# shenwei356/wfa

Hardware: AMD Instinct MI355X
Metric: aligned pairs/sec (and Gcells/s) on 1e6 synthetic 1 kbp pairs @5% error (higher is better)
Workload: dtype u32; 1 GPU; 1000000 x 1000 bp pairs/GPU @5% error, global gap-affine 4/6/2, wf-adaptive 10/50/1, seed 3; config=c3, pairs_per_gpu=1000000, length=1000, parallelism=pair-sharded x1, ranks_seen_by_collective=1, backend=none (1 GPU), collective_forced=False, status_ok=1000000, setup_steps=0, gather=none (1 GPU), gather_bytes_per_rank_step=0, packed_pairs=1000000, retried_pairs=832

## Files before the change

wfa_amd/csrc/wfa_ctx.hpp:

```cpp
#pragma once
#include "../../include/wfa_hip.h"
#include "wfa_common.hpp"

#include <algorithm>
#include <atomic>
#include <chrono>
#include <cmath>
#include <cstdio>
#include <cstdlib>
#include <cstring>
#include <deque>
#include <functional>
#include <malloc.h>
#include <mutex>
#include <new>
#include <numeric>
#include <string>
#include <thread>
#include <vector>
#include <fcntl.h>
#include <optional>
#include <sys/file.h>
#include <unistd.h>

// ... 105 lines not shown
    int64_t       opt_team_slack           = 1024;
    bool          dbg_teamc                = false;
    DevBuf        xbuf;
    int64_t       opt_team_paged           = 1;
    DevBuf        page_ctl;
    int64_t       opt_team_xcd             = 2;
    int64_t       opt_arena_poison         = 0;
    int64_t       opt_pilot                = 1;
    int64_t       opt_tail_overlap         = 1;
    int64_t       opt_overlap              = 0;
    int64_t       opt_fail_pass            = 0;
    int64_t       opt_prepack              = 0;
    int64_t       opt_narrow_long          = 0;
    DevBuf        score_out;
    DevBuf        wide_ckpt;
    DevBuf        mx_seq, mx_words;
    DevBuf        sd_ctl, sd_blk, sd_list, sd_redo;
    uint64_t      sd_n_words = 0, sd_n_listed = 0;
    DevBuf        mx_out;
    uint2        *mx_pin       = nullptr;
    size_t        mx_pin_bytes = 0;
    hipEvent_t    mx_ev[4]     = {};
    int64_t       opt_matrix_tile_cells    = 0;
    int64_t       opt_score_long_min       = 64;
    int64_t       opt_score_long_window    = 256;
    int64_t       opt_wide                 = 1;
    int64_t       opt_wide_max_len         = 2047;
    int           opt_wide_waves           = 0;
    bool          opt_wide_exact           = false;
    int64_t       opt_wide_min_pairs       = 64;
    int64_t       opt_duo                  = 1;
    int64_t       opt_duo_min_pairs        = 200000;
    bool          opt_duo_pk               = true;
    int64_t       opt_duo_short            = 0;
    int64_t       opt_duo_short_min_pairs  = 50000;
    bool          ctrl_clean               = false;
    hipStream_t   ctrl_clean_stream        = nullptr;
    hipEvent_t    ctrl_clean_ev            = nullptr;
    bool          redo_was_empty           = false;
    int64_t       opt_compact_call_bases   = 50000000;
    int64_t       opt_lane                 = 1;
    int64_t       opt_lane_pack            = 1;
    int64_t       opt_lane_min_pairs       = 32768;
    int64_t       opt_long                 = 1;
    int64_t       opt_long_min_len         = 4000;
    int64_t       opt_long_window_words    = 240;
    int64_t       opt_long_first           = 0;
    int64_t       opt_long_wave_bt         = 1;
    int64_t       opt_census               = 0;
    int64_t       opt_learn                = 1;
    uint64_t      learn_key                = 0;
    int           learn_level              = 0;
    uint32_t      learn_calls              = 0;
    uint64_t      rows_key                 = 0;
    uint32_t      rows_scale               = 1;
    uint64_t      band_key                 = 0;
    int           band_kind                = 0;
    uint32_t      band_calls               = 0;
    int64_t       opt_blk_mid              = 1;
    int64_t       opt_mem_limit            = 0;
    int           force_mode               = -1;
    const uint32_t *dbg_arena = nullptr;
    const uint4    *dbg_meta  = nullptr;
    uint64_t        dbg_words = 0, dbg_first = 0, dbg_n = 0;
    uint32_t        dbg_fmt = 0, dbg_g = 1;
    wfahip_timing timing{};
// ... 49 lines not shown
```

wfa_amd/csrc/wfa_duo.hip:

```cpp
#define WFA_NO_AUX_KERNELS 1
#include "wfa_duo.hpp"
#include "wfa_fwd.hpp"

namespace wfa {

namespace {
template <int DX, int DOE>
hipError_t go_duo(const KParams &P, uint32_t grid, size_t lds_bytes, hipStream_t st, bool census, bool pk) {
    if (pk && census)
        hipLaunchKernelGGL((wfa_duo_kernel<true, DX, DOE>), dim3(grid), dim3(64), lds_bytes, st, P);
    else if (pk)
        hipLaunchKernelGGL((wfa_duo_kernel<false, DX, DOE>), dim3(grid), dim3(64), lds_bytes, st, P);
    else if (census)
        hipLaunchKernelGGL((wfa_duo32_kernel<true, DX, DOE>), dim3(grid), dim3(64), lds_bytes, st, P);
    else
        hipLaunchKernelGGL((wfa_duo32_kernel<false, DX, DOE>), dim3(grid), dim3(64), lds_bytes, st, P);
    return hipGetLastError();
}
}

hipError_t wfa_launch_duo(int shape, const KParams &P, uint32_t grid, size_t lds_bytes, hipStream_t st, bool census, bool pk) {
    switch (shape) {
    case 0: return go_duo<2, 4>(P, grid, lds_bytes, st, census, pk);
    case 1: return go_duo<1, 3>(P, grid, lds_bytes, st, census, pk);
    case 2: return go_duo<1, 2>(P, grid, lds_bytes, st, census, pk);
    case 3: return go_duo<2, 3>(P, grid, lds_bytes, st, census, pk);
    case 4: return go_duo<2, 2>(P, grid, lds_bytes, st, census, pk);
    case 5: return go_duo<3, 3>(P, grid, lds_bytes, st, census, pk);
    }
    return hipErrorInvalidValue;
}

}
```

wfa_amd/csrc/wfa_duo.hpp:

```cpp
#pragma once
#include "wfa_blk.hpp"
#include "wfa_duo_cfg.hpp"
#include "wfa_pk16.hpp"

namespace wfa {

struct DuoRed {
#define WFA_DUO_3(opa, opb, opc)                                                                                    \
    unsigned long long sv;                                                                                          \
    asm volatile("s_nop 1\n\t" opa " %0, %0, %0 " WFA_DPP_CTL_XOR1 "\n\t" opb " %1, %1, %1 " WFA_DPP_CTL_XOR1 "\n\t" opc \
        " %2, %2, %2 " WFA_DPP_CTL_XOR1 "\n\t" opa " %0, %0, %0 " WFA_DPP_CTL_XOR2 "\n\t" opb " %1, %1, %1 "        \
        WFA_DPP_CTL_XOR2 "\n\t" opc " %2, %2, %2 " WFA_DPP_CTL_XOR2 "\n\t" opa " %0, %0, %0 " WFA_DPP_CTL_HMIR "\n\t" \
        opb " %1, %1, %1 " WFA_DPP_CTL_HMIR "\n\t" opc " %2, %2, %2 " WFA_DPP_CTL_HMIR "\n\t"                         \
        "s_and_saveexec_b64 %3, %4\n\t" opa " %0, %0, %0 " WFA_DPP_CTL_MIR "\n\t" opb " %1, %1, %1 " WFA_DPP_CTL_MIR    \
        "\n\t" opc " %2, %2, %2 " WFA_DPP_CTL_MIR "\n\ts_mov_b64 exec, %3"                                            \
        : "+v"(a), "+v"(b), "+v"(c), "=&s"(sv)                                                                      \
        : "s"(wm)                                                                                                   \
        : "scc");
#define WFA_DUO_2(opa, opb)                                                                                         \
    unsigned long long sv;                                                                                          \
    asm volatile("s_nop 1\n\t" opa " %0, %0, %0 " WFA_DPP_CTL_XOR1 "\n\t" opb " %1, %1, %1 " WFA_DPP_CTL_XOR1 "\n\ts_nop 0\n\t" \
        opa " %0, %0, %0 " WFA_DPP_CTL_XOR2 "\n\t" opb " %1, %1, %1 " WFA_DPP_CTL_XOR2 "\n\ts_nop 0\n\t" opa        \
        " %0, %0, %0 " WFA_DPP_CTL_HMIR "\n\t" opb " %1, %1, %1 " WFA_DPP_CTL_HMIR "\n\t"                            \
        "s_and_saveexec_b64 %2, %3\n\t" opa " %0, %0, %0 " WFA_DPP_CTL_MIR "\n\t" opb " %1, %1, %1 " WFA_DPP_CTL_MIR    \
        "\n\ts_mov_b64 exec, %2"                                                                                    \
        : "+v"(a), "+v"(b), "=&s"(sv)                                                                               \
        : "s"(wm)                                                                                                   \
        : "scc");
#define WFA_DUO_1(opa)                                                                                              \
    unsigned long long sv;                                                                                          \
    asm volatile("s_nop 1\n\t" opa " %0, %0, %0 " WFA_DPP_CTL_XOR1 "\n\ts_nop 1\n\t" opa " %0, %0, %0 " WFA_DPP_CTL_XOR2 \
        "\n\ts_nop 1\n\t" opa " %0, %0, %0 " WFA_DPP_CTL_HMIR "\n\t"                                                \
        "s_and_saveexec_b64 %1, %2\n\ts_nop 0\n\t" opa " %0, %0, %0 " WFA_DPP_CTL_MIR "\n\ts_mov_b64 exec, %1"       \
        : "+v"(a), "=&s"(sv)                                                                                        \
        : "s"(wm)                                                                                                   \
        : "scc");
    static WFA_DEV void min_max_min(int &a, int &b, int &c, unsigned long long wm) { WFA_DUO_3("v_min_i32_dpp", "v_max_i32_dpp", "v_min_i32_dpp") }
    static WFA_DEV void min_max(int &a, int &b, unsigned long long wm) { WFA_DUO_2("v_min_i32_dpp", "v_max_i32_dpp") }
    static WFA_DEV void max_add(int &a, int &b, unsigned long long wm) { WFA_DUO_2("v_max_i32_dpp", "v_add_u32_dpp") }
    static WFA_DEV int  max1(int a, unsigned long long wm) {
        WFA_DUO_1("v_max_i32_dpp")
        return a;
    }
    static WFA_DEV int or1(int a, unsigned long long wm) {
        WFA_DUO_1("v_or_b32_dpp")
        return a;
    }
#undef WFA_DUO_3
#undef WFA_DUO_2
#undef WFA_DUO_1
};

template <bool CENSUS, int DX, int DOE, bool PK>
__device__ __attribute__((always_inline)) inline void duo_run(const KParams &P) {
    constexpr int PP = 4;
    static_assert(DX >= 1 && DOE >= 1 && DX <= 4 && DOE <= 4, "ring depths of one to four score steps");
    constexpr int R  = DX > DOE ? DX : DOE;
    constexpr int RW = PK ? 2 : PP;
    extern __shared__ __attribute__((aligned(16))) uint32_t lds[];
    const int  lane = threadIdx.x, l7 = lane & 7, l15 = lane & 15;
    const bool hi_half = (lane & 8) != 0;

    const uint32_t  SW = P.lds_seq_words, PW = P.prepack_words;
    const uint32_t  FP = duo_fetch_pairs(PW), NBUF = duo_bufs(PW);
    uint32_t *const park0 = lds + NBUF * PW;
    const uint64_t  cap      = P.arena_words;
    const int       mdd      = (int)P.max_dist_diff;
    const int       minwf    = (int)P.min_wf_len;
    const bool      adaptive = P.adaptive != 0;
    const uint32_t  seed_si  = P.dx;
    uint32_t        pk_one   = 0x00010001u;
    if constexpr (PK) asm volatile("" : "+s"(pk_one));
    const int       rows_cap = (int)(cap / 32);

    int       st = 0;
    bool      wide = false;
    uint32_t  pidx = 0, si = 0, cells = 0, sbuf = 0;
    int       n = 0, m = 0, kb = 0;
    bool      slow = false, first_eq = false;
    int             j = l7, k0 = 0;
    uint32_t        mdn = 0u, mup = 0u;
    const uint32_t *lq = lds + 4, *lt = lds + 4;
    uint32_t       *rowp = nullptr;

    uint32_t M[R][RW], I[RW], D[RW];
    int      rlo[R], rhi[R];
    int      lim[PP], lmx[PP];
#pragma unroll
    for (int d = 0; d < R; d++) {
        rlo[d] = BK_BIG, rhi[d] = -BK_BIG;
#pragma unroll
        for (int p = 0; p < RW; p++) M[d][p] = 0u;
    }
#pragma unroll
    for (int p = 0; p < RW; p++) I[p] = D[p] = 0u;
#pragma unroll
    for (int p = 0; p < PP; p++) lim[p] = 0, lmx[p] = 0;

    uint32_t buf_free  = (1u << NBUF) - 1u;
    uint32_t park_used = 0u;
    constexpr uint32_t PF_TOK = 1u, PF_LD = 2u, PF_STAGED = 4u, PF_DRY = 8u;
    uint32_t pf = 0u;
    uint32_t pf_tok = 0u, pf_ld_idx = 0u, pf_idx = 0u, pf_buf = 0u;
    uint32_t st_mask = 0u;
    uint4    pf_w = make_uint4(0u, 0u, 0u, 0u);

#ifdef WFA_STAMPS
    unsigned long long stamp_acc[8] = {0, 0, 0, 0, 0, 0, 0, 0}, stamp_prev;
    unsigned long long evt[8] = {0, 0, 0, 0, 0, 0, 0, 0};
    asm volatile("s_memtime %0\n\ts_waitcnt lgkmcnt(0)" : "=s"(stamp_prev)::"memory");
#endif
    const auto pair_of = [&](uint32_t idx) { return P.work ? P.work[idx] : P.chunk_first + idx; };
    const auto dn1 = [&](uint32_t x) { return (uint32_t)__builtin_amdgcn_update_dpp(0, (int)x, 0x111, 0xf, 0xf, true) & mdn; };
    const auto up1 = [&](uint32_t x) { return (uint32_t)__builtin_amdgcn_update_dpp(0, (int)x, 0x101, 0xf, 0xf, true) & mup; };
    const auto other_half = [&](int x) { return __builtin_amdgcn_update_dpp(0, x, 0x128, 0xf, 0xf, true); };
    const auto set_derived = [&]() {
        j   = wide ? l15 : l7;
        mdn = j == 0 ? 0u : ~0u;
        mup = j == (wide ? 15 : 7) ? 0u : ~0u;
        k0  = kb + PP * j;
#pragma unroll
        for (int p = 0; p < PP; p++) lim[p] = imax2(1, imin2(n + k0 + p, m)), lmx[p] = imax2(n + k0 + p, m);
        lq   = lds + sbuf * PW + 4u;
        lt   = lq + SW;
        if constexpr (DUO_ARENA_FMT == 10u)
            rowp = P.arena + (uint64_t)pidx * cap + (((uint32_t)k0 & 56u) >> 3) * (uint32_t)(rows_cap * 4) + (((uint32_t)k0 >> 2) & 1u) * 16u;
        else if constexpr (DUO_ARENA_FMT == 9u)
            rowp = P.arena + (uint64_t)pidx * cap + (((uint32_t)k0 & 60u) >> 2) * (uint32_t)(rows_cap * 2) + si * 2u;
        else
            rowp = P.arena + (uint64_t)pidx * cap + (uint64_t)(si >> 3) * 256u + (si & 7u) * 2u;
    };
    const auto clear_rings = [&]() {
#pragma unroll
        for (int d = 0; d < R; d++) {
            rlo[d] = BK_BIG, rhi[d] = -BK_BIG;
#pragma unroll
            for (int p = 0; p < RW; p++) M[d][p] = 0u;
        }
#pragma unroll
        for (int p = 0; p < RW; p++) I[p] = D[p] = 0u;
    };
    const auto or_halves = [&](uint32_t v) {
        uint32_t r = 0u;
#pragma unroll
        for (int o = 0; o < 8; o++) r |= (uint32_t)__builtin_amdgcn_readlane((int)v, 8 * o);
        return r;
    };

    const auto refill = [&](auto ph_c) __attribute__((always_inline)) -> bool {
        constexpr int ph  = decltype(ph_c)::value;
        constexpr int NEW = (ph + R - 1) % R;
        pf        = (uint32_t)__builtin_amdgcn_readfirstlane((int)pf);
        park_used = (uint32_t)__builtin_amdgcn_readfirstlane((int)park_used);
        buf_free  = (uint32_t)__builtin_amdgcn_readfirstlane((int)buf_free);
        st_mask   = (uint32_t)__builtin_amdgcn_readfirstlane((int)st_mask);
        if ((pf & (PF_LD | PF_STAGED)) == PF_LD) {
            const uint32_t cnt = umin2(FP, P.chunk_n - pf_ld_idx);
            st_mask = 0u;
            {
                uint32_t f = buf_free;
                for (uint32_t c = 0; c < cnt; c++) st_mask |= f & (0u - f), f &= f - 1u;
            }
            buf_free &= ~st_mask;
            const uint32_t w0 = (uint32_t)lane * 4u, slot = w0 / PW;
            if (slot < cnt) {
                uint32_t f = st_mask;
                for (uint32_t c = 0; c < slot; c++) f &= f - 1u;
                const uint32_t b = (uint32_t)__builtin_ctz(f);
                *reinterpret_cast<uint4 *>(lds + b * PW + (w0 - slot * PW)) = pf_w;
            }
            pf_idx = pf_ld_idx, pf = (pf | PF_STAGED) & ~PF_LD;
        }
        if ((pf & (PF_TOK | PF_LD)) == PF_TOK) {
            pf_ld_idx = (uint32_t)__builtin_amdgcn_readfirstlane((int)pf_tok);
            const bool have = pf_ld_idx < P.chunk_n;
            if (have) {
                const uint32_t *const slot = P.prepack + (uint64_t)pf_ld_idx * PW;
                const uint32_t cnt = umin2(FP, P.chunk_n - pf_ld_idx);
                if ((uint32_t)lane * 4u < cnt * PW) pf_w = *reinterpret_cast<const uint4 *>(slot + lane * 4);
            }
            pf = (pf & ~PF_TOK) | (have ? PF_LD : PF_DRY);
        }
        if ((pf & (PF_TOK | PF_DRY)) == 0u) {
            if (lane == 0) pf_tok = atomicAdd(P.queue_head, FP);
            pf |= PF_TOK;
        }
        unsigned long long m_free;
        WFA_STAMP(0);
        for (;;) {
        const bool run   = st == 1;
        const int  Wc    = wide ? 64 : 32;
        const bool touch = run && rhi[NEW] >= rlo[NEW] && (rlo[NEW] <= kb || rhi[NEW] >= kb + Wc - 1);
        bool       narrowable = false;
        if constexpr (ph == 0) {
            int ulo = rlo[0], uhi = rhi[0];
#pragma unroll
            for (int d = 1; d < R; d++) ulo = imin2(ulo, rlo[d]), uhi = imax2(uhi, rhi[d]);
            narrowable    = run && wide && uhi - ulo + 1 <= DUO_NARROW_AT;
        }
        const unsigned long long m_ev = __ballot(touch || narrowable);
        m_free = __ballot(st == 0);
        if (__builtin_expect(!(m_ev != 0ull || (m_free != 0ull && (park_used != 0u || (pf & PF_STAGED) != 0u))), 1)) break;
        WFA_EVT(1, 1);
        {
            int ulo = rlo[0], uhi = rhi[0];
#pragma unroll
// ... 177 lines not shown
                const uint32_t this_idx = pf_idx;
                pf_idx += 1u;
                const uint32_t *const hb = lds + pf_buf * PW;
                const uint32_t nq = (uint32_t)__builtin_amdgcn_readfirstlane((int)hb[0]), mt = (uint32_t)__builtin_amdgcn_readfirstlane((int)hb[1]);
                const uint32_t status = (uint32_t)__builtin_amdgcn_readfirstlane((int)hb[2]);
                if (st_mask == 0u) pf &= ~PF_STAGED;
                if (status != ST_PENDING) {
                    if (lane == 0) {
                        P.pair_meta[this_idx] = make_uint4(status, 0u, 0u, 0u);
                        if (status >= ST_REDO_BYTES) push_redo(P, pair_of(this_idx), status);
                    }
                    buf_free |= 1u << pf_buf;
                    continue;
                }
                WFA_EVT(5, 1);
                if (mine) {
                    pidx = this_idx, sbuf = pf_buf;
                    n = (int)nq, m = (int)mt;
                    const int Ak = m - n;
                    si = 0, cells = 0, slow = false;
                    kb = -16 + PP * imax2(-3, imin2(3, Ak / (2 * PP)));
                    first_eq = ((hb[4] ^ hb[4 + SW]) & 3u) == 0u;
                    clear_rings();
                    st = 1, wide = false;
                }
                m_free &= ~(0xFFull << (8 * oct));
            }
            set_derived();
            __builtin_amdgcn_fence(__ATOMIC_RELEASE, "wavefront");
            __builtin_amdgcn_fence(__ATOMIC_ACQUIRE, "wavefront");
        }
        }
        WFA_STAMP(1);
        return m_free == ~0ull && park_used == 0u && (pf & (PF_DRY | PF_LD | PF_STAGED)) == PF_DRY;
    };

    const auto step = [&](auto ph_c) __attribute__((always_inline)) {
        constexpr int ph = decltype(ph_c)::value;
        const bool run = (st == 1);
        const unsigned long long wm = __ballot(wide);
        WFA_EVT(0, 1), WFA_EVT(6, __builtin_popcountll(__ballot(run)) / 8);

        uint32_t(&Mo)[RW] = M[(ph + R - DOE) % R];
        uint32_t(&Mx)[RW] = M[(ph + R - DX) % R];
        uint32_t(&Mn)[RW] = M[ph];

        uint32_t nM[PP], nI[RW], nD[RW], wd[RW], cc[PP];
        const uint32_t a_edge = dn1(Mo[RW - 1]), b_edge = dn1(I[RW - 1]);
        const uint32_t c_edge = up1(Mo[0]), d_edge = up1(D[0]);
        const bool     slow_any = __ballot(run && slow) != 0ull;
        const auto next_slow = [&](const uint32_t(&Mo4)[PP], const uint32_t(&I4)[PP], const uint32_t(&D4)[PP], const uint32_t(&Mx4)[PP],
                                   uint32_t ae, uint32_t be, uint32_t ce, uint32_t de, uint32_t(&nI4)[PP], uint32_t(&nD4)[PP],
                                   uint32_t(&wd4)[PP]) __attribute__((always_inline)) {
#pragma unroll
            for (int p = 0; p < PP; p++) {
                const int      k  = k0 + p;
                const uint32_t a0 = p ? Mo4[p - 1] : ae, b0 = p ? I4[p - 1] : be;
                const uint32_t c0 = p < PP - 1 ? Mo4[p + 1] : ce, d0 = p < PP - 1 ? D4[p + 1] : de;
                const uint32_t x0 = Mx4[p];
                const uint32_t a = (int)a0 > m ? 0u : a0, b = (int)b0 > m ? 0u : b0;
                const uint32_t c = (int)c0 - k > n ? 0u : c0, d = (int)d0 - k > n ? 0u : d0;
                const uint32_t x = ((int)x0 > m || (int)x0 - k > n) ? 0u : x0;
                const uint32_t mi = umax2(a, b), tI = umin2(mi, 1u), Isk = mi + tI;
                const uint32_t Dsk = umax2(c, d), tD = umin2(Dsk, 1u);
                const uint32_t x1  = x + umin2(x, 1u);
                const uint32_t Msk = umax3(Isk, Dsk, x1);
                const bool fromX = x != 0u && Msk == x1;
// ... 267 lines not shown
        if (run && !fin) si += 1u;
        WFA_STAMP(5);
    };

    for (;;) {
        if (refill(std::integral_constant<int, 0>{})) break;
        step(std::integral_constant<int, 0>{});
        if constexpr (R > 1) {
            if (refill(std::integral_constant<int, 1 % R>{})) break;
            step(std::integral_constant<int, 1 % R>{});
        }
        if constexpr (R > 2) {
            if (refill(std::integral_constant<int, 2 % R>{})) break;
            step(std::integral_constant<int, 2 % R>{});
        }
        if constexpr (R > 3) {
            if (refill(std::integral_constant<int, 3 % R>{})) break;
            step(std::integral_constant<int, 3 % R>{});
        }
    }
#ifdef WFA_STAMPS
    if (lane == 0 && P.debug_info) {
        unsigned long long *acc = reinterpret_cast<unsigned long long *>(P.debug_info);
        for (int i = 0; i < 8; i++) atomicAdd(acc + i, stamp_acc[i]);
        for (int i = 0; i < 8; i++) atomicAdd(acc + 8 + i, evt[i]);
    }
#endif
}

#ifndef WFA_DUO_VGPRS
#define WFA_DUO_VGPRS 64
#endif
static_assert(16u * (256u - 4u) / 2u < 2048u, "wfa_duo_kernel's packed rings need offsets under 4 096");
template <bool CENSUS, int DX = 2, int DOE = 4>
__global__ __launch_bounds__(64, WFA_DUO_WAVES) __attribute__((amdgpu_num_vgpr(WFA_DUO_VGPRS))) void wfa_duo_kernel(const KParams P) {
    duo_run<CENSUS, DX, DOE, true>(P);
}
template <bool CENSUS, int DX = 2, int DOE = 4>
__global__ __launch_bounds__(64, WFA_DUO_WAVES) __attribute__((amdgpu_num_vgpr(WFA_DUO_VGPRS))) void wfa_duo32_kernel(const KParams P) {
    duo_run<CENSUS, DX, DOE, false>(P);
}

}
```

wfa_amd/csrc/wfa_duo_cfg.hpp:

```cpp
#pragma once
#include "wfa_common.hpp"

namespace wfa {

#ifndef WFA_DUO_WAVES
#define WFA_DUO_WAVES 4
#endif
#ifndef WFA_DUO_PARK
#define WFA_DUO_PARK 4
#endif
#ifndef WFA_DUO_WIDEN_AT
#define WFA_DUO_WIDEN_AT 26
#endif
#ifndef WFA_DUO_NARROW_AT
#define WFA_DUO_NARROW_AT 21
#endif
#ifndef WFA_DUO_GROUP_MAJOR
#define WFA_DUO_GROUP_MAJOR 2
#endif
constexpr uint32_t DUO_ARENA_FMT = WFA_DUO_GROUP_MAJOR == 2 ? 10u : WFA_DUO_GROUP_MAJOR == 1 ? 9u : 7u;
constexpr int DUO_PARK       = WFA_DUO_PARK;
constexpr int DUO_PARK_WORDS = 8 * 12 + 16;
constexpr int DUO_BUFS       = 8 + 1 + DUO_PARK;
constexpr int DUO_FETCH_MAX  = 8;
constexpr int DUO_WIDEN_AT   = WFA_DUO_WIDEN_AT;
constexpr int DUO_NARROW_AT  = WFA_DUO_NARROW_AT;
constexpr int DUO_WIDE_MAX   = 56;

__host__ __device__ inline uint32_t duo_fetch_pairs(uint32_t prepack_words) {
    const uint32_t f = 256u / prepack_words;
    return f < 1u ? 1u : (f > (uint32_t)DUO_FETCH_MAX ? (uint32_t)DUO_FETCH_MAX : f);
}
__host__ __device__ inline uint32_t duo_bufs(uint32_t prepack_words) { return 8u + duo_fetch_pairs(prepack_words) + (uint32_t)DUO_PARK; }
__host__ __device__ inline uint32_t duo_lds_words(uint32_t prepack_words) {
    return duo_bufs(prepack_words) * prepack_words + (uint32_t)DUO_PARK * DUO_PARK_WORDS;
}

hipError_t wfa_launch_duo(int shape, const KParams &P, uint32_t grid, size_t lds_bytes, hipStream_t st, bool census, bool pk);

}
```

wfa_amd/csrc/wfa_host.hip:

```cpp
#include <map>
#include "wfa_ctx.hpp"
#include "wfa_generic.hpp"
#include "wfa_packed.hpp"
#include "wfa_reg.hpp"
#include "wfa_blk.hpp"
#include "wfa_duo_cfg.hpp"
#include "wfa_lane.hpp"
#include "wfa_team.hpp"
#include "wfa_teamc.hpp"
#include "wfa_fwd.hpp"
#include "wfa_long.hpp"
#include "wfa_wide.hpp"

using namespace wfa;
static_assert(TEAM_SOLO_MAX == 4096, "wfa_ctx.hpp: default of opt_team_solo_max");

namespace wfa {
hipError_t wfa_launch_fwd(int shape, int kind, uint32_t flags, const KParams &P, uint32_t grid, size_t lds_bytes, hipStream_t st) {
    switch (shape) {
    case 0: return wfa_launch_fwd_s24(kind, flags, P, grid, lds_bytes, st);
    case 1: return wfa_launch_fwd_s13(kind, flags, P, grid, lds_bytes, st);
    case 2: return wfa_launch_fwd_s12(kind, flags, P, grid, lds_bytes, st);
    case 3: return wfa_launch_fwd_s23(kind, flags, P, grid, lds_bytes, st);
    case 4: return wfa_launch_fwd_s22(kind, flags, P, grid, lds_bytes, st);
// ... 376 lines not shown
        ctx->opt_long_first = value;
    else if (k == "long_wave_bt_pairs")
        ctx->opt_long_wave_bt_pairs = value;
    else if (k == "long_mid_lone")
        ctx->opt_long_mid_lone = value;
    else if (k == "pair_lds")
        ctx->opt_pair_lds = value, ctx->one_lds_skip = 0;
    else if (k == "long_wave_bt")
        ctx->opt_long_wave_bt = value;
    else if (k == "long_min_len")
        ctx->opt_long_min_len = value;
    else if (k == "long_window_words")
        ctx->opt_long_window_words = (value >= 64 && value <= 4096 && value % 4 == 0) ? value : 240;
    else if (k == "wide")
        ctx->opt_wide = value;
    else if (k == "wide_min_pairs")
        ctx->opt_wide_min_pairs = value;
    else if (k == "matrix_tile_cells")
        ctx->opt_matrix_tile_cells = value > 0 ? value : 0;
    else if (k == "score_long_min")
        ctx->opt_score_long_min = value > 0 ? value : 1;
    else if (k == "score_long_window_words")
        ctx->opt_score_long_window = value;
    else if (k == "wide_max_len")
        ctx->opt_wide_max_len = value;
    else if (k == "wide_exact")
        ctx->opt_wide_exact = value != 0;
    else if (k == "wide_waves")
        ctx->opt_wide_waves = (value == 1 || value == 4) ? (int)value : 0;
    else if (k == "duo")
        ctx->opt_duo = value;
    else if (k == "duo_pk")
        ctx->opt_duo_pk = value != 0;
    else if (k == "duo_min_pairs")
        ctx->opt_duo_min_pairs = value;
    else if (k == "compact_call_bases")
        ctx->opt_compact_call_bases = value;
    else if (k == "lane")
        ctx->opt_lane = value;
    else if (k == "lane_pack")
        ctx->opt_lane_pack = value;
    else if (k == "lane_min_pairs")
        ctx->opt_lane_min_pairs = value;
    else if (k == "duo_short")
        ctx->opt_duo_short = value;
    else if (k == "duo_short_min_pairs")
        ctx->opt_duo_short_min_pairs = value;
    else if (k == "blk_mid")
        ctx->opt_blk_mid = value;
    else if (k == "pair_fast")
        ctx->opt_pair_fast = value;
    else if (k == "arena_budget_pct")
        ctx->opt_arena_budget_pct = value;
    else if (k == "autopack")
        ctx->opt_autopack = value;
    else if (k == "learn")
        ctx->opt_learn = value, ctx->learn_key = 0;
    else if (k == "mem_limit") {
        ctx->opt_mem_limit = value;
        hipDeviceProp_t prop;
        if (value > 0)
            ctx->total_mem = (size_t)value;
        else if (hipGetDeviceProperties(&prop, ctx->device) == hipSuccess)
            ctx->total_mem = prop.totalGlobalMem;
    }
    else
// ... 316 lines not shown
            if (overlap && count >= 8 * resident) chunk = std::min<uint64_t>(chunk, (count + 7) / 8);
            if (ctx->opt_chunk_pairs > 0) chunk = std::min<uint64_t>(chunk, (uint64_t)ctx->opt_chunk_pairs);
            const uint64_t n_chunks = (count + chunk - 1) / chunk;
            const uint32_t n_buf    = (overlap && n_chunks > 1) ? 2 : 1;
            const uint64_t chunk_alloc = list ? std::max<uint64_t>(chunk, std::min<uint64_t>(chunk + chunk / 4 + 64, budget / (words * 4ull))) : chunk;
            int rc2 = WFAHIP_OK;
            if (arena_buf.bytes < (size_t)(words * 4ull * chunk * n_buf)) {
                rc2 = ensure(ctx, arena_buf, (size_t)(words * 4ull * chunk_alloc * n_buf));
                if (rc2 == WFAHIP_ERR_OOM && chunk_alloc > chunk) rc2 = ensure(ctx, arena_buf, (size_t)(words * 4ull * chunk * n_buf));
            }
            if (rc2) return rc2;
            if (meta_buf.bytes < chunk * 16 * n_buf && (rc2 = ensure(ctx, meta_buf, chunk_alloc * 16 * n_buf))) return rc2;
            detach_bt = detach_bt && n_chunks == 1 && ctx->opt_tail_overlap != 0 &&
                        (count * (uint64_t)max_len > (uint64_t)ctx->opt_compact_call_bases || ctx->opt_compact_call_bases <= 0);
            ctrl_fresh = false;
            const bool stream_bt = kind == 3 && shape == 0 && !blk_batch && n_buf == 1 && ctx->opt_bt_stream > 0 && (int64_t)chunk >= ctx->opt_bt_stream_min &&
                                   ctx->opt_bt_stream_single != 0;
            P.done_q = nullptr, P.done_ctl = nullptr, P.n_stream_wgs = 0;
            if (stream_bt) {
                if ((rc2 = ensure(ctx, ctx->doneq, 256 + 16 * chunk))) return rc2;
                P.done_ctl = static_cast<uint32_t *>(ctx->doneq.p);
                P.done_q   = reinterpret_cast<uint4 *>(static_cast<char *>(ctx->doneq.p) + 256);
            }
            ctx->timing.arena_bytes = std::max<uint64_t>(ctx->timing.arena_bytes, words * 4ull * chunk * n_buf);
            if (list && (rc2 = upload_work(list->data(), count))) return rc2;
            while (ctx->evpool.size() < 4 * n_chunks) {
                hipEvent_t e;
                HIP_TRY(hipEventCreate(&e));
                ctx->evpool.push_back(e);
            }
            if (!ctrl_zeroed) HIP_TRY(hipMemsetAsync(d_ctrl, 0, 8, st));
            ctrl_zeroed = false;
            hipStream_t st_bt = (n_buf == 2 || detach_bt) ? ctx->stream2 : st;
            for (uint64_t c = 0; c < n_chunks; c++) {
                const uint64_t c0 = c * chunk, cn = std::min<uint64_t>(chunk, count - c0);
                hipEvent_t evFa = ctx->evpool[4 * c], evFb = ctx->evpool[4 * c + 1];
                hipEvent_t evBa = detach_bt ? ctx->evBtA : ctx->evpool[4 * c + 2];
                hipEvent_t evBb = detach_bt ? ctx->evBtB : ctx->evpool[4 * c + 3];
                const uint32_t buf = (uint32_t)(c % n_buf);
                P.arena       = static_cast<uint32_t *>(arena_buf.p) + (uint64_t)buf * chunk * words;
                P.pair_meta   = static_cast<uint4 *>(meta_buf.p) + (uint64_t)buf * chunk;
                P.chunk_first = (uint32_t)(first_pair + c0), P.chunk_n = (uint32_t)cn;
                P.work        = list ? static_cast<const uint32_t *>(ctx->work.p) + c0 : nullptr;
                if (!list && c == 0 && first_pair == 0)
                    ctx->dbg_arena = P.arena, ctx->dbg_meta = P.pair_meta, ctx->dbg_words = words, ctx->dbg_first = first_pair,
                    ctx->dbg_n = cn, ctx->dbg_fmt = P.compact_fmt, ctx->dbg_g = P.g;
                uint32_t grid = (uint32_t)std::min<uint64_t>((uint64_t)ctx->num_cus * waves_per_cu,
                                                            (cn + pairs_wave - 1) / pairs_wave);
                const uint32_t n_bt = stream_bt ? (uint32_t)std::min<int64_t>(ctx->opt_bt_stream, grid / 4) : 0u;
                if (stream_bt) {
                    if (grid < (uint32_t)ctx->num_cus * waves_per_cu) grid = std::min<uint32_t>(grid + n_bt, (uint32_t)ctx->num_cus * waves_per_cu);
                    P.n_stream_wgs = n_bt;
                    P.stream_wait  = (uint32_t)std::min<int64_t>(std::max<int64_t>(ctx->opt_bt_stream_wait_us, 0) * 100, 0x7FFFFFFF);
                    HIP_TRY(hipMemsetAsync(ctx->doneq.p, 0, 256 + 16 * cn, st));
                    HIP_TRY(hipMemsetAsync(P.pair_meta, 0xFF, 16 * cn, st));
                }
                P.prepack = nullptr, P.prepack_words = 0;
                P.lds_seq_words = is_long ? long_sw : kind == 10 ? lane_sw : kind == 8 ? duo_sw : seq_words;
                if (kind == 10) P.sub_lds_words = lane_stride_words(lane_sw);
                if ((kind == 3 && !blk_batch && !list && ctx->opt_prepack != 0) || kind == 8 || (kind == 10 && ctx->opt_lane_pack == 0) || is_long) {
                    const uint32_t pw = 4u + 2u * P.lds_seq_words;
                    if ((rc2 = ensure(ctx, ctx->prepack, (size_t)chunk * pw * 4))) return rc2;
                    if (ctx->pk_words)
                        hipLaunchKernelGGL(wfa_prepack_words_kernel, dim3((uint32_t)((cn + 3) / 4)), dim3(256), 0, st, P, ctx->pk_words,
                                           static_cast<uint32_t *>(ctx->prepack.p), P.lds_seq_words, pw);
                    else {
                        const uint32_t ppw = (cn <= (uint64_t)ctx->num_cus * 64 && 2u * P.lds_seq_words > 32u) ? 1u : (uint32_t)PREPACK_PAIRS;
                        hipLaunchKernelGGL(wfa_prepack_kernel, dim3((uint32_t)((cn + 4 * ppw - 1) / (4 * ppw))), dim3(256), 0, st, P,
                                           static_cast<uint32_t *>(ctx->prepack.p), P.lds_seq_words, pw, ppw);
                    }
                    HIP_TRY(hipGetLastError());
                    P.prepack = static_cast<const uint32_t *>(ctx->prepack.p), P.prepack_words = pw;
                } else if (ctx->pk_words) {
                    hipLaunchKernelGGL(wfa_unpack_pairs_kernel, dim3((uint32_t)((cn + 3) / 4)), dim3(256), 0, st, P, ctx->pk_words,
                                       const_cast<uint8_t *>(P.blob));
                    HIP_TRY(hipGetLastError());
                }
                if (is_long) P.lds_seq_words = long_cw;
                if (n_buf == 2 && c >= 2) HIP_TRY(hipStreamWaitEvent(st, ctx->evpool[4 * (c - 2) + 3], 0));
                if (c > 0) HIP_TRY(hipMemsetAsync(d_ctrl, 0, 4, st));
                if (ctx->opt_arena_poison) HIP_TRY(hipMemsetAsync(P.arena, 0xA5, (size_t)(words * 4ull * cn), st));
                HIP_TRY(hipEventRecord(evFa, st));
                if (kind == 8) {
                    HIP_TRY(wfa_launch_duo(shape, P, grid, lds_bytes, st, P.census != 0, ctx->opt_duo_pk));
                } else if (kind >= 3) {
                    uint32_t fl = (P.census ? (uint32_t)FWD_CENSUS : 0u) | (P.adaptive ? (uint32_t)FWD_ADAPTIVE : 0u);
                    if (kind == 3 && stream_bt) fl |= FWD_STREAM;
                    if (blk_batch) {
                        const uint64_t groups = (uint64_t)ctx->num_cus * 16 * pairs_wave;
                        const uint64_t share  = (cn + groups - 1) / groups;
                        const uint64_t rounds = (share + BLK_BATCH - 1) / BLK_BATCH;
                        P.blk_batch_n = (uint32_t)std::min<uint64_t>(BLK_BATCH, std::max<uint64_t>(1, (share + rounds - 1) / std::max<uint64_t>(1, rounds)));
                        if (ctx->opt_blk_batch > 1) P.blk_batch_n = (uint32_t)std::min<int64_t>(BLK_BATCH, ctx->opt_blk_batch);
                        fl |= FWD_BATCH;
                    }
                    HIP_TRY(wfa_launch_fwd(shape, kind, fl, P, grid, lds_bytes, st));
                } else if (kind == 2)
                    hipLaunchKernelGGL((wfa_reg_kernel<2, 4, 1>), dim3(grid), dim3(64), lds_bytes, st, P);
                else
                    hipLaunchKernelGGL(wfa_packed_kernel, dim3(grid), dim3(64), lds_bytes, st, P);
                HIP_TRY(hipGetLastError());
                HIP_TRY(hipEventRecord(evFb, st));
                if (st_bt != st) HIP_TRY(hipStreamWaitEvent(st_bt, evFb, 0));
                if (st_bt != st) HIP_TRY(hipEventRecord(evBa, st_bt));
                if (is_long && (ctx->opt_long_wave_bt >= 2 || (ctx->opt_long_wave_bt == 1 && cn <= (ctx->opt_long_wave_bt_pairs ? (uint64_t)ctx->opt_long_wave_bt_pairs : (uint64_t)ctx->num_cus * 20))))
                    hipLaunchKernelGGL(wfa_backtrace_wave_kernel, dim3((uint32_t)((cn + BTW_WAVES - 1) / BTW_WAVES)), dim3(64 * BTW_WAVES), 0, st_bt, P);
                else
                    hipLaunchKernelGGL(wfa_backtrace_kernel, dim3((uint32_t)((cn + BT_THREADS - 1) / BT_THREADS)), dim3(BT_THREADS), 0, st_bt, P);
                HIP_TRY(hipGetLastError());
                HIP_TRY(hipEventRecord(evBb, st_bt));
            }
            if (st_bt != st && !detach_bt)
                for (uint64_t c = (n_chunks >= 2 ? n_chunks - 2 : 0); c < n_chunks; c++)
                    HIP_TRY(hipStreamWaitEvent(st, ctx->evpool[4 * c + 3], 0));
            uint32_t hc[CTRL_WORDS];
            if (!detach_bt) HIP_TRY(hipEventRecord(ctx->ev1, st));
            if ((rc2 = fetch_ctrl(hc, &redo_out))) return rc2;
            if (detach_bt) ctx->bt_pending = true;
            else ctrl_fresh = true, std::memcpy(hc_last, hc, sizeof hc_last);
            for (uint64_t c = 0; c < n_chunks; c++) {
                float msF = 0, msB = 0;
                HIP_TRY(hipEventElapsedTime(&msF, ctx->evpool[4 * c], ctx->evpool[4 * c + 1]));
                if (!detach_bt) HIP_TRY(hipEventElapsedTime(&msB, ctx->evpool[4 * c + (st_bt != st ? 2 : 1)], ctx->evpool[4 * c + 3]));
                ctx->timing.kernel_ms += msF + msB;
                if (!list) ctx->timing.main_kernel_ms += msF, ctx->timing.n_main_launches++;
                ctx->timing.n_launches += 2;
            }
            P.work = nullptr;
            P.lds_seq_words = seq_words;
            P.sub_lds_words = (uint32_t)sub_words;
            return WFAHIP_OK;
        };

        if (can_b || can_c || can_d) {
            std::vector<uint64_t> redo1, redo2;
            const bool narrow1 = can_d && ctx->opt_blk == 16 && ctx->opt_blk_narrow != 0 &&
                                 ((ctx->opt_blk_batch != 0 && max_len < 200 && seq_words <= 16) ||
                                  (ctx->opt_narrow_long != 0 && shape == 0 && (size_t)seq_words * 2 * 4 * 8 + 16 <= 8 * 1024));
            const bool duo_long  = !narrow1 && seq_words > 16 &&
                                   (ctx->opt_duo >= 2 || (ctx->opt_duo == 1 && (int64_t)n_pairs >= ctx->opt_duo_min_pairs));
            const bool duo_short = seq_words <= 16 && ctx->opt_duo != 0 &&
                                   (ctx->opt_duo_short >= 2 || (ctx->opt_duo_short == 1 && (int64_t)n_pairs >= ctx->opt_duo_short_min_pairs));
            const bool duo1    = can_d && ctx->opt_blk == 16 && (duo_long || duo_short) && 4u + 2u * ((seq_words + 1u) & ~1u) <= 256u;
            const bool lane1   = can_d && ctx->opt_blk == 16 && seq_words <= (uint32_t)LN_SEQ_WORDS &&
                                 (ctx->opt_lane >= 2 || (ctx->opt_lane == 1 && (int64_t)n_pairs >= ctx->opt_lane_min_pairs));
            const int  kind1   = long_first ? 11 : (duo1 && duo_short) ? 8 : lane1 ? 10 : duo1 ? 8 : narrow1 ? 6 : (can_d ? (ctx->opt_blk == 8 ? 4 : 3) : (can_c ? 2 : 1));
            const int  kind_mid = long_first ? 12 : 9, kind_wide = long_first ? 13 : 5, kind_64 = long_first ? 11 : 3;
            uint64_t done_pairs = 0;
            bool     skip_rest  = false;
            int      kind_rest  = kind1;
            const bool wide_ok  = kind1 >= 3 && ctx->opt_blk_wide != 0;
            std::vector<uint64_t> redo_w;
            uint64_t mid_in = 0, mid_fail = 0;
            const auto wide_pass = [&](std::vector<uint64_t> &from, bool from_mid = false) -> int {
                std::vector<uint32_t> lst;
                for (uint64_t e : from) {
                    if ((uint32_t)(e >> 32) == ST_REDO_BAND) lst.push_back((uint32_t)e);
                    else redo_w.push_back(e);
                }
                from.clear();
// ... 626 lines not shown
```

Baseline: 62.74 million pairs/s.

## Fuse raw-byte prepacking into duo kernel prefetch pipeline

Adds a RAW mode to the duo kernel. In this mode each wave reads the pair header (lengths and offsets) and the raw ASCII bases straight from the blob, packs them to 2-bit words in registers and stages them in LDS. This removes the separate prepack kernel launch and its intermediate global buffer. The prefetch state machine gains header, load and late-stage phases, plus a fast path for aligned sequences of 16–1024 bases, and falls back to a REDO_BYTES status on invalid characters. It is on by default for the duo path when the fetch batch is one pair. The cost is more VGPR pressure and scalar-branch overhead inside the main kernel.

```diff
diff --git a/wfa_amd/csrc/wfa_ctx.hpp b/wfa_amd/csrc/wfa_ctx.hpp
--- a/wfa_amd/csrc/wfa_ctx.hpp
+++ b/wfa_amd/csrc/wfa_ctx.hpp
@@ -161,6 +161,7 @@
     int64_t       opt_duo                  = 1;
     int64_t       opt_duo_min_pairs        = 200000;
     bool          opt_duo_pk               = true;
+    bool          opt_duo_raw              = true;
     int64_t       opt_duo_short            = 0;
     int64_t       opt_duo_short_min_pairs  = 50000;
     bool          ctrl_clean               = false;
diff --git a/wfa_amd/csrc/wfa_duo.hip b/wfa_amd/csrc/wfa_duo.hip
--- a/wfa_amd/csrc/wfa_duo.hip
+++ b/wfa_amd/csrc/wfa_duo.hip
@@ -6,8 +6,13 @@
 
 namespace {
 template <int DX, int DOE>
-hipError_t go_duo(const KParams &P, uint32_t grid, size_t lds_bytes, hipStream_t st, bool census, bool pk) {
-    if (pk && census)
+hipError_t go_duo(const KParams &P, uint32_t grid, size_t lds_bytes, hipStream_t st, bool census, bool pk, bool raw) {
+    if (raw && !pk) return hipErrorInvalidValue;
+    if (raw && census)
+        hipLaunchKernelGGL((wfa_duo_kernel<true, DX, DOE, true>), dim3(grid), dim3(64), lds_bytes, st, P);
+    else if (raw)
+        hipLaunchKernelGGL((wfa_duo_kernel<false, DX, DOE, true>), dim3(grid), dim3(64), lds_bytes, st, P);
+    else if (pk && census)
         hipLaunchKernelGGL((wfa_duo_kernel<true, DX, DOE>), dim3(grid), dim3(64), lds_bytes, st, P);
     else if (pk)
         hipLaunchKernelGGL((wfa_duo_kernel<false, DX, DOE>), dim3(grid), dim3(64), lds_bytes, st, P);
@@ -19,14 +24,14 @@
 }
 }
 
-hipError_t wfa_launch_duo(int shape, const KParams &P, uint32_t grid, size_t lds_bytes, hipStream_t st, bool census, bool pk) {
+hipError_t wfa_launch_duo(int shape, const KParams &P, uint32_t grid, size_t lds_bytes, hipStream_t st, bool census, bool pk, bool raw) {
     switch (shape) {
-    case 0: return go_duo<2, 4>(P, grid, lds_bytes, st, census, pk);
-    case 1: return go_duo<1, 3>(P, grid, lds_bytes, st, census, pk);
-    case 2: return go_duo<1, 2>(P, grid, lds_bytes, st, census, pk);
-    case 3: return go_duo<2, 3>(P, grid, lds_bytes, st, census, pk);
-    case 4: return go_duo<2, 2>(P, grid, lds_bytes, st, census, pk);
-    case 5: return go_duo<3, 3>(P, grid, lds_bytes, st, census, pk);
+    case 0: return go_duo<2, 4>(P, grid, lds_bytes, st, census, pk, raw);
+    case 1: return go_duo<1, 3>(P, grid, lds_bytes, st, census, pk, raw);
+    case 2: return go_duo<1, 2>(P, grid, lds_bytes, st, census, pk, raw);
+    case 3: return go_duo<2, 3>(P, grid, lds_bytes, st, census, pk, raw);
+    case 4: return go_duo<2, 2>(P, grid, lds_bytes, st, census, pk, raw);
+    case 5: return go_duo<3, 3>(P, grid, lds_bytes, st, census, pk, raw);
     }
     return hipErrorInvalidValue;
 }
diff --git a/wfa_amd/csrc/wfa_duo.hpp b/wfa_amd/csrc/wfa_duo.hpp
--- a/wfa_amd/csrc/wfa_duo.hpp
+++ b/wfa_amd/csrc/wfa_duo.hpp
@@ -51,7 +51,30 @@
 #undef WFA_DUO_1
 };
 
-template <bool CENSUS, int DX, int DOE, bool PK>
+WFA_DEV uint32_t raw_start(uint32_t len, uint32_t l16) { return umin2(l16, len - 16u); }
+WFA_DEV uint4 raw_load16(const uint8_t *p) {
+    uint4 v;
+    __builtin_memcpy(&v, p, 16);
+    return v;
+}
+WFA_DEV uint32_t raw_pack16(const uint4 &v, uint32_t len, uint32_t l16, bool &bad) {
+    const uint32_t r[4] = {v.x, v.y, v.z, v.w};
+    uint32_t       word = 0u;
+#pragma unroll
+    for (int i = 0; i < 4; i++) {
+        const uint32_t x = (r[i] >> 1) & 0x03030303u;
+        bad |= __builtin_amdgcn_perm(0u, 0x47544341u, x) != r[i];
+        uint32_t a, b;
+        asm("v_lshl_add_u32 %0, %1, 6, %1" : "=v"(a) : "v"(x));
+        asm("v_lshl_add_u32 %0, %1, 12, %1" : "=v"(b) : "v"(a));
+        word |= ((b >> 18) & 0xFFu) << (8 * i);
+    }
+    uint32_t rest;
+    asm("v_sub_u32_e64 %0, %1, %2 clamp" : "=v"(rest) : "s"(len), "v"(l16));
+    return (uint32_t)((uint64_t)word >> (32u - 2u * umin2(rest, 16u)));
+}
+
+template <bool CENSUS, int DX, int DOE, bool PK, bool RAW = false>
 __device__ __attribute__((always_inline)) inline void duo_run(const KParams &P) {
     constexpr int PP = 4;
     static_assert(DX >= 1 && DOE >= 1 && DX <= 4 && DOE <= 4, "ring depths of one to four score steps");
@@ -62,7 +85,7 @@
     const bool hi_half = (lane & 8) != 0;
 
     const uint32_t  SW = P.lds_seq_words, PW = P.prepack_words;
-    const uint32_t  FP = duo_fetch_pairs(PW), NBUF = duo_bufs(PW);
+    const uint32_t  FP = RAW ? 1u : duo_fetch_pairs(PW), NBUF = duo_bufs(PW);
     uint32_t *const park0 = lds + NBUF * PW;
     const uint64_t  cap      = P.arena_words;
     const int       mdd      = (int)P.max_dist_diff;
@@ -99,11 +122,26 @@
 
     uint32_t buf_free  = (1u << NBUF) - 1u;
     uint32_t park_used = 0u;
+    constexpr uint32_t PF_HD = 16u, PF_LT = 32u, PF_BAD = 64u, PF_FAST = 128u;
     constexpr uint32_t PF_TOK = 1u, PF_LD = 2u, PF_STAGED = 4u, PF_DRY = 8u;
     uint32_t pf = 0u;
     uint32_t pf_tok = 0u, pf_ld_idx = 0u, pf_idx = 0u, pf_buf = 0u;
     uint32_t st_mask = 0u;
     uint4    pf_w = make_uint4(0u, 0u, 0u, 0u);
+    uint32_t pf_h = 0u, pf_hd = 0u, pf_hd_idx = 0u;
+    const auto raw_hd   = [](uint32_t h, int i) { return (uint32_t)__builtin_amdgcn_readlane((int)h, i); };
+    const auto raw_hd64 = [&](uint32_t h, int i) { return raw_hd(h, i) | ((uint64_t)raw_hd(h, i + 1) << 32); };
+    const auto raw_status = [&](uint32_t nq, uint32_t mt) -> uint32_t {
+        if (nq == 0 || mt == 0) return ST_EMPTY;
+        if (nq > 0x1FFFFFFFu || mt > 0x1FFFFFFFu) return ST_TOO_LONG;
+        if (((nq > mt ? nq : mt) + 15u) / 16u + 1u > SW) return ST_REDO_LDS;
+        return ST_PENDING;
+    };
+    const auto raw_lane = [&]() {
+        uint32_t l = (uint32_t)lane;
+        asm volatile("" : "+v"(l));
+        return l;
+    };
 
 #ifdef WFA_STAMPS
     unsigned long long stamp_acc[8] = {0, 0, 0, 0, 0, 0, 0, 0}, stamp_prev;
@@ -154,7 +192,43 @@
         park_used = (uint32_t)__builtin_amdgcn_readfirstlane((int)park_used);
         buf_free  = (uint32_t)__builtin_amdgcn_readfirstlane((int)buf_free);
         st_mask   = (uint32_t)__builtin_amdgcn_readfirstlane((int)st_mask);
-        if ((pf & (PF_LD | PF_STAGED)) == PF_LD) {
+        if (RAW && (pf & PF_LT) != 0u) {
+            const uint32_t  nq = raw_hd(pf_hd, 0), mt = raw_hd(pf_hd, 1), ln = raw_lane();
+            uint32_t        status = raw_status(nq, mt);
+            uint32_t *const sl     = lds + (uint32_t)__builtin_ctz(st_mask) * PW;
+            bool            bad    = false;
+            if (__builtin_expect((pf & PF_FAST) != 0u, 1)) {
+                const uint32_t tw = raw_pack16(pf_w, mt, ln * 16u, bad);
+                if (ln < SW) sl[4u + SW + ln] = tw;
+                if (ln + 64u < SW) sl[4u + SW + 64u + ln] = 0u;
+            } else if (status == ST_PENDING) {
+                const uint64_t qo = raw_hd64(pf_hd, 2), to = raw_hd64(pf_hd, 4);
+                for (uint32_t v = ln; v < 2u * SW; v += 64u) {
+                    const bool isq = v < SW;
+                    sl[4u + v]     = prepack_word(P.blob, isq ? qo : to, isq ? nq : mt, isq ? v : v - SW, bad);
+                }
+            }
+            if (__ballot(bad) != 0ull || (pf & PF_BAD) != 0u) status = ST_REDO_BYTES;
+            if (ln == 0u) *reinterpret_cast<uint4 *>(sl) = make_uint4(nq, mt, status, 0u);
+            pf_idx = pf_ld_idx, pf = (pf | PF_STAGED) & ~(PF_LT | PF_BAD | PF_FAST);
+        }
+        if (RAW && (pf & (PF_LD | PF_LT | PF_STAGED)) == PF_LD) {
+            st_mask = buf_free & (0u - buf_free);
+            buf_free &= ~st_mask;
+            if ((pf & PF_FAST) != 0u) {
+                const uint32_t  nq = raw_hd(pf_hd, 0), mt = raw_hd(pf_hd, 1), ln = raw_lane(), l16 = ln * 16u;
+                const uint64_t  to = raw_hd64(pf_hd, 4);
+                uint32_t *const sl = lds + (uint32_t)__builtin_ctz(st_mask) * PW;
+                bool            bad = false;
+                const uint32_t  qw  = raw_pack16(pf_w, nq, l16, bad);
+                pf_w = raw_load16(P.blob + to + raw_start(mt, l16));
+                if (ln < SW) sl[4u + ln] = qw;
+                if (ln + 64u < SW) sl[4u + 64u + ln] = 0u;
+                if (__ballot(bad) != 0ull) pf |= PF_BAD;
+            }
+            pf = (pf | PF_LT) & ~PF_LD;
+        }
+        if (!RAW && (pf & (PF_LD | PF_STAGED)) == PF_LD) {
             const uint32_t cnt = umin2(FP, P.chunk_n - pf_ld_idx);
             st_mask = 0u;
             {
@@ -171,7 +245,28 @@
             }
             pf_idx = pf_ld_idx, pf = (pf | PF_STAGED) & ~PF_LD;
         }
-        if ((pf & (PF_TOK | PF_LD)) == PF_TOK) {
+        if (RAW && (pf & (PF_HD | PF_LD | PF_LT)) == PF_HD) {
+            const uint32_t nq = raw_hd(pf_h, 0), mt = raw_hd(pf_h, 1);
+            const uint64_t qo = raw_hd64(pf_h, 2), to = raw_hd64(pf_h, 4);
+            const uint64_t base = (uint64_t)(uintptr_t)P.blob;
+            const bool     fast = raw_status(nq, mt) == ST_PENDING && nq - 16u <= 1008u && mt - 16u <= 1008u && (((base + qo) | (base + to)) & 15ull) == 0ull;
+            if (fast) pf_w = raw_load16(P.blob + qo + raw_start(nq, raw_lane() * 16u));
+            pf_hd = pf_h, pf_ld_idx = pf_hd_idx;
+            pf = (pf & ~PF_HD) | PF_LD | (fast ? PF_FAST : 0u);
+        }
+        if (RAW && (pf & (PF_TOK | PF_HD)) == PF_TOK) {
+            pf_hd_idx = (uint32_t)__builtin_amdgcn_readfirstlane((int)pf_tok);
+            const bool have = pf_hd_idx < P.chunk_n;
+            const uint32_t ln = raw_lane();
+            if (have && ln < 6u) {
+                const uint32_t *const hp = ln == 0u   ? P.q_len
+                                           : ln == 1u ? P.t_len
+                                                      : reinterpret_cast<const uint32_t *>(ln < 4u ? P.q_off : P.t_off) + (ln & 1u);
+                pf_h = hp[(uint64_t)(P.chunk_first + pf_hd_idx) << (ln < 2u ? 0 : 1)];
+            }
+            pf = (pf & ~PF_TOK) | (have ? PF_HD : PF_DRY);
+        }
+        if (!RAW && (pf & (PF_TOK | PF_LD)) == PF_TOK) {
             pf_ld_idx = (uint32_t)__builtin_amdgcn_readfirstlane((int)pf_tok);
             const bool have = pf_ld_idx < P.chunk_n;
             if (have) {
@@ -415,7 +510,7 @@
         }
         }
         WFA_STAMP(1);
-        return m_free == ~0ull && park_used == 0u && (pf & (PF_DRY | PF_LD | PF_STAGED)) == PF_DRY;
+        return m_free == ~0ull && park_used == 0u && (pf & (PF_DRY | PF_HD | PF_LD | PF_LT | PF_STAGED)) == PF_DRY;
     };
 
     const auto step = [&](auto ph_c) __attribute__((always_inline)) {
@@ -749,9 +844,9 @@
 #define WFA_DUO_VGPRS 64
 #endif
 static_assert(16u * (256u - 4u) / 2u < 2048u, "wfa_duo_kernel's packed rings need offsets under 4 096");
-template <bool CENSUS, int DX = 2, int DOE = 4>
+template <bool CENSUS, int DX = 2, int DOE = 4, bool RAW = false>
 __global__ __launch_bounds__(64, WFA_DUO_WAVES) __attribute__((amdgpu_num_vgpr(WFA_DUO_VGPRS))) void wfa_duo_kernel(const KParams P) {
-    duo_run<CENSUS, DX, DOE, true>(P);
+    duo_run<CENSUS, DX, DOE, true, RAW>(P);
 }
 template <bool CENSUS, int DX = 2, int DOE = 4>
 __global__ __launch_bounds__(64, WFA_DUO_WAVES) __attribute__((amdgpu_num_vgpr(WFA_DUO_VGPRS))) void wfa_duo32_kernel(const KParams P) {
diff --git a/wfa_amd/csrc/wfa_duo_cfg.hpp b/wfa_amd/csrc/wfa_duo_cfg.hpp
--- a/wfa_amd/csrc/wfa_duo_cfg.hpp
+++ b/wfa_amd/csrc/wfa_duo_cfg.hpp
@@ -36,6 +36,6 @@
     return duo_bufs(prepack_words) * prepack_words + (uint32_t)DUO_PARK * DUO_PARK_WORDS;
 }
 
-hipError_t wfa_launch_duo(int shape, const KParams &P, uint32_t grid, size_t lds_bytes, hipStream_t st, bool census, bool pk);
+hipError_t wfa_launch_duo(int shape, const KParams &P, uint32_t grid, size_t lds_bytes, hipStream_t st, bool census, bool pk, bool raw);
 
 }
diff --git a/wfa_amd/csrc/wfa_host.hip b/wfa_amd/csrc/wfa_host.hip
--- a/wfa_amd/csrc/wfa_host.hip
+++ b/wfa_amd/csrc/wfa_host.hip
@@ -432,6 +432,8 @@
         ctx->opt_duo = value;
     else if (k == "duo_pk")
         ctx->opt_duo_pk = value != 0;
+    else if (k == "duo_raw")
+        ctx->opt_duo_raw = value != 0;
     else if (k == "duo_min_pairs")
         ctx->opt_duo_min_pairs = value;
     else if (k == "compact_call_bases")
@@ -814,6 +816,7 @@
             if (!ctrl_zeroed) HIP_TRY(hipMemsetAsync(d_ctrl, 0, 8, st));
             ctrl_zeroed = false;
             hipStream_t st_bt = (n_buf == 2 || detach_bt) ? ctx->stream2 : st;
+            uint32_t    n_pack_launches = 0;
             for (uint64_t c = 0; c < n_chunks; c++) {
                 const uint64_t c0 = c * chunk, cn = std::min<uint64_t>(chunk, count - c0);
                 hipEvent_t evFa = ctx->evpool[4 * c], evFb = ctx->evpool[4 * c + 1];
@@ -840,8 +843,12 @@
                 P.prepack = nullptr, P.prepack_words = 0;
                 P.lds_seq_words = is_long ? long_sw : kind == 10 ? lane_sw : kind == 8 ? duo_sw : seq_words;
                 if (kind == 10) P.sub_lds_words = lane_stride_words(lane_sw);
-                if ((kind == 3 && !blk_batch && !list && ctx->opt_prepack != 0) || kind == 8 || (kind == 10 && ctx->opt_lane_pack == 0) || is_long) {
+                const bool duo_raw = kind == 8 && ctx->opt_duo_raw && ctx->opt_duo_pk && !ctx->pk_words && !list && duo_fetch_pairs(duo_pw) == 1u;
+                if (duo_raw) {
+                    P.prepack_words = duo_pw;
+                } else if ((kind == 3 && !blk_batch && !list && ctx->opt_prepack != 0) || kind == 8 || (kind == 10 && ctx->opt_lane_pack == 0) || is_long) {
                     const uint32_t pw = 4u + 2u * P.lds_seq_words;
+                    n_pack_launches++;
                     if ((rc2 = ensure(ctx, ctx->prepack, (size_t)chunk * pw * 4))) return rc2;
                     if (ctx->pk_words)
                         hipLaunchKernelGGL(wfa_prepack_words_kernel, dim3((uint32_t)((cn + 3) / 4)), dim3(256), 0, st, P, ctx->pk_words,
@@ -864,7 +871,7 @@
                 if (ctx->opt_arena_poison) HIP_TRY(hipMemsetAsync(P.arena, 0xA5, (size_t)(words * 4ull * cn), st));
                 HIP_TRY(hipEventRecord(evFa, st));
                 if (kind == 8) {
-                    HIP_TRY(wfa_launch_duo(shape, P, grid, lds_bytes, st, P.census != 0, ctx->opt_duo_pk));
+                    HIP_TRY(wfa_launch_duo(shape, P, grid, lds_bytes, st, P.census != 0, ctx->opt_duo_pk, duo_raw));
                 } else if (kind >= 3) {
                     uint32_t fl = (P.census ? (uint32_t)FWD_CENSUS : 0u) | (P.adaptive ? (uint32_t)FWD_ADAPTIVE : 0u);
                     if (kind == 3 && stream_bt) fl |= FWD_STREAM;
@@ -908,6 +915,7 @@
                 if (!list) ctx->timing.main_kernel_ms += msF, ctx->timing.n_main_launches++;
                 ctx->timing.n_launches += 2;
             }
+            ctx->timing.n_launches += n_pack_launches;
             P.work = nullptr;
             P.lds_seq_words = seq_words;
             P.sub_lds_words = (uint32_t)sub_words;
```

Result: no change. 63.15 million pairs/s, median of 6 (+0.7%).
